# balazs-bamer/cdpr-simulation

Measured on AMD Instinct MI355X. Metric: CDPR sim-steps/sec (whole node), 65 536 parallel 8-cable robots, 1 ms dt, higher is better.
Workload: dtype f32

## Files before the change

cdpr-simulation_amd/csrc/cdpr_engine_launch.hip:

```cpp
#include "cdpr_engine_internal.hpp"

namespace cdpr_host {

double sim_time(uint64_t step, double dt) {
  const int64_t dt_ns = (int64_t)std::llround(dt * 1e9);
  const int64_t now_ns = (int64_t)step * dt_ns;
  return (double)(now_ns / 1000000000LL) + (double)(now_ns % 1000000000LL) * 1e-9;
}

uint64_t publish_mask(const cdpr_engine* h, int k, double& last) {
  uint64_t mask = 0;
  last = h->prev_publish;
  if (h->cfg.publish_period == 0.0) {
    if (k > 0 && h->step + (uint64_t)k > 1) last = sim_time(h->step + (uint64_t)k - 1, h->cfg.dt);
    mask = (k >= 64) ? ~0ull : ((1ull << k) - 1ull);
    return h->step == 0 ? (mask & ~1ull) : mask;
  }
  for (int j = 0; j < k; ++j) {
    const double now = sim_time(h->step + (uint64_t)j, h->cfg.dt);
    if ((now - last) > h->cfg.publish_period) {
      last = now;
      if (j < 64) mask |= (1ull << j);
    }
  }
  return mask;
}

void advance_clock(cdpr_engine* h, int k, int launches) {
  (void)publish_mask(h, k, h->prev_publish);
  if (!h->plan.general && h->mode != kModeForce) h->pid_calls = sat_pid_calls(h->pid_calls + k - (h->step == 0 ? 1 : 0));
  h->step += (uint64_t)k;
  h->launches += (uint64_t)launches;
}

static void set_weight_row(const cdpr_engine* h, StepArgs& a, int slot) {
  memcpy(a.wrow, &h->wtab_host[(h->plan.per_robot || h->mode == kModeVelocity) ? 0 : 1][slot * (kWin + 2)], sizeof a.wrow);
}

LaunchShape launch_shape(const cdpr_engine* h, int k, bool steady, const Schedule* sched) {
  LaunchShape s;
  s.steps = k;
  s.first_world = h->step == 0;
  s.scheduled = sched != nullptr;
  s.steady = steady;
  return s;
}
StepKernel step_kernel_of(const cdpr_engine* h, const PlannedKernel& pk) {
  const uint32_t n = h->n;
  switch (pk.id) {
    case KernelId::StepSingle: return pick_step_kernel(true, n, h->plan.fk, h->plan.td);
    case KernelId::StepMulti: return pick_step_kernel(false, n, h->plan.fk, h->plan.td);
    case KernelId::Lowreg: return pick_lowreg_kernel(n, h->plan.td);
    case KernelId::OnestepPersist: return pick_onestep_persist_kernel(n, h->plan.fk, h->plan.td);
    case KernelId::Split: return pick_split_kernel(n);
    case KernelId::Onestep: return pick_onestep_kernel(n, h->plan.fk, h->plan.td);
    case KernelId::PhysStep: return pick_phys_kernel(n, h->plan.fk, h->plan.td, kPhysStep);
    case KernelId::Rollout: return pick_rollout_kernel(n, h->plan.fk, h->plan.td);
    case KernelId::PhysRollout: return pick_phys_kernel(n, h->plan.fk, h->plan.td, kPhysRollout);
    case KernelId::PrSingle: return pick_pr_kernel(true, false, false, n, h->plan.fk, h->plan.td);
    case KernelId::PrLowreg: return pick_pr_kernel(true, false, true, n, h->plan.fk, h->plan.td);
    case KernelId::PrSplit: return pick_pr_split_kernel(n);
    case KernelId::PrMulti: return pick_pr_kernel(false, false, false, n, h->plan.fk, h->plan.td);
    case KernelId::PrRollout: return pick_pr_kernel(false, true, false, n, h->plan.fk, h->plan.td);
    case KernelId::PairSingle: return pick_pair_kernel(true, n, h->plan.fk, h->plan.td);
    case KernelId::PairMulti: return pick_pair_kernel(false, n, h->plan.fk, h->plan.td);
    case KernelId::PairStream: return pick_pair_stream_kernel(n, h->mode == kModeVelocity);
    case KernelId::Cable: return pick_cable_kernel(n, h->plan.fk, h->plan.td);
    default: return nullptr;
  }
}
StepKernel select_step_kernel(const cdpr_engine* h, int k, bool steady) { return step_kernel_of(h, planned_kernel(h->plan, launch_shape(h, k, steady))); }
static bool pair_stream_steady(const cdpr_engine* h, const StepArgs& a, const Schedule* sched) {
  return h->step != 0 && h->mode != kModeForce && a.pid_calls >= a.nbuf && h->cfg.publish_period == 0.0 && !a.dbg && !a.travel_on &&
         !(a.vel_limit > 0.f) && !a.unilateral && a.effort >= 0.f && a.clamp_cmd && !(sched && sched->ready);
}
static bool split_steady_launch(const cdpr_engine* h, const PlannedKernel& pk, const StepArgs& a) {
  return pk.id == KernelId::Split && h->split_steady && !h->plan.per_robot && h->step != 0 && h->mode != kModeForce && a.pid_calls != 0 &&
         a.pid_calls >= a.nbuf && h->cfg.publish_period == 0.0 && !a.dbg && !a.travel_on;
}
uint32_t step_block_threads(const cdpr_engine* h, int k) { return planned_kernel(h->plan, launch_shape(h, k)).block; }

static StepArgs handle_args(const cdpr_engine* h, const void* record) {
  StepArgs a = h->base;
  a.state = h->d_state;
  a.obs = h->d_obs;
  a.dbg = h->dbg ? h->d_dbg : nullptr;
  a.geom = h->d_geom;
  a.batch = h->batch;
  a.stride = h->stride;
  a.obs_step_stride = record ? (size_t)h->n_obs * h->stride : 0;
  return a;
}

static StepArgs fast_path_args(const cdpr_engine* h, const void* record, const Schedule* sched) {
  StepArgs a = handle_args(h, record);
  if (h->plan.per_robot) {
    copy_pid(h->pid_vel, a);
    copy_pid_alt(h->pid_pos, a.alt);
    a.cmd = h->d_target;
    a.meta = h->d_mode;
  } else {
    copy_pid(h->mode == kModeVelocity ? h->pid_vel : h->pid_pos, a);
    a.cmd = h->cmd[cmd_kind_of_mode(h->mode)].latched();
    a.flags = h->mode == kModeVelocity ? kFlagActualIsVelocity : h->mode == kModeForce ? kFlagForceMode : 0u;
  }
  if (sched) {
    a.flags |= kFlagPublishAll;
    a.sched_refresh = sched->refresh;
    a.sched_stride = (size_t)h->batch * h->n;
    a.sched_ready = sched->ready;
    a.fault = sched->fault;
  }
  return a;
}

int warm_first_launch(cdpr_engine* h) {
  if (h->plan.general || h->plan.fp64) return CDPR_OK;
  if (const char* w = std::getenv("CDPR_NO_WARM_LAUNCH"))
    if (w[0] == '1') return CDPR_OK;
  const uint32_t rows = 64;
  const std::vector<float4> s = home_state(h, rows);
  DevBuf st, ob, cm, mt;
  HIP_TRY(h, mt.alloc(rows));
  HIP_TRY(h, hipMemsetAsync(mt.p, (int)(kMetaPosition | (20u << kMetaCallShift)), rows, h->stream));
  HIP_TRY(h, st.alloc(s.size() * sizeof(float4)));
  HIP_TRY(h, ob.alloc((size_t)h->n_obs * rows * sizeof(float4)));
  HIP_TRY(h, cm.alloc((size_t)rows * h->n * sizeof(float)));
  HIP_TRY(h, hipMemcpyAsync(st.p, s.data(), s.size() * sizeof(float4), hipMemcpyHostToDevice, h->stream));
  HIP_TRY(h, hipMemsetAsync(cm.p, 0, (size_t)rows * h->n * sizeof(float), h->stream));
  StepArgs a = h->base;
  a.state = st.as<float4>();
  a.obs = ob.as<float4>();
  a.cmd = cm.as<float>();
  a.dbg = nullptr;
  a.geom = h->d_geom;
  a.batch = h->plan.lane_cable ? (h->n <= 4 ? 16u : 8u) : h->plan.lane_pair ? 32u : 64u;
  a.stride = rows;
  a.nsteps = 1;
  a.obs_step_stride = 0;
  a.flags = 0u;
  a.publish_mask = 1ull;
  copy_pid(h->plan.per_robot ? h->pid_vel : h->pid_pos, a);
  copy_pid_alt(h->pid_pos, a.alt);
  a.meta = mt.as<uint8_t>();
  a.pid_calls = kCallSat;
  a.ring_slot = 0;
  set_weight_row(h, a, 0);
  hipLaunchKernelGGL(select_step_kernel(h, 1), dim3(1), dim3(step_block_threads(h, 1)), 0, h->stream, a);
  HIP_TRY(h, hipGetLastError());
  if (planned_kernel(h->plan, launch_shape(h, 1)).id == KernelId::Split && h->split_steady) {
    for (const bool vel : {false, true}) {
      copy_pid(vel ? h->pid_vel : h->pid_pos, a);
      hipLaunchKernelGGL(pick_split_steady_kernel(h->n, vel), dim3(1), dim3(128), 0, h->stream, a);
      HIP_TRY(h, hipGetLastError());
    }
  }
  HIP_TRY(h, wait_stream(h));
  return CDPR_OK;
}

static int launch_step(cdpr_engine* h, StepKernel kern, uint32_t robots_per_block, dim3 block, const StepArgs& a, uint32_t max_grid = 0) {
  const uint32_t B = a.batch;
  const uint32_t chunk = (h->plan.chunk && B > h->plan.chunk) ? h->plan.chunk : B;
  const uint32_t pieces = (B + chunk - 1u) / chunk;
  const uint32_t each = (((B + pieces - 1u) / pieces) + 63u) & ~63u;
  int launches = 0;
  for (uint32_t first = 0; first < B; first += each, ++launches) {
    StepArgs c = a;
    c.batch = std::min(each, B - first);
    c.state = a.state + first;
    c.obs = a.obs + first;
    if (a.cmd) c.cmd = a.cmd + (size_t)first * h->n;
    if (a.dbg) c.dbg = a.dbg + (size_t)first * CDPR_PID_DEBUG_AXES;
    if (a.meta) c.meta = a.meta + first;
    uint32_t grid = (c.batch + robots_per_block - 1u) / robots_per_block;
    if (max_grid && grid > max_grid) grid = max_grid;
    hipLaunchKernelGGL(kern, dim3(grid), block, 0, h->stream, c);
  }
  return launches;
}

static void flush_hot(cdpr_engine* h) {
  if (!h->d_rec || !h->plan.gen_hot) return;
  GenFlushArgs fa{};
  fa.rec = h->d_rec, fa.rstride = h->stride, fa.batch = h->batch, fa.lay = h->glay, fa.nbuf = std::max(h->gpid[0].nbuf, 1);
  hipLaunchKernelGGL(cdpr_gen_flush_hot_kernel, dim3((h->batch + 255u) / 256u), dim3(256), 0, h->stream, fa);
}

static hipError_t reset_block(cdpr_engine* h, int which) {
  const GenLayout& L = h->glay;
  flush_hot(h);
  hipError_t e1 = hipMemsetAsync(h->d_rec + (size_t)L.block_a(which, 0) * h->stride * 4, 0, (size_t)L.pid_slots() * h->stride * 16, h->stream);
  if (e1 != hipSuccess || L.pid_rows() == 0) return e1;
  return hipMemsetAsync(h->d_rec + ((size_t)L.slots() * 4 + (size_t)L.block_b(which, 0)) * h->stride, 0, (size_t)L.pid_rows() * h->stride * 4, h->stream);
}

static hipError_t reset_block64(cdpr_engine* h, int which) {
  for (uint32_t i = 0; i < h->n; ++i) {
    hipError_t e1 = hipMemsetAsync(h->d_state64 + (size_t)f64_hold_row((int)h->n, (int)i, which, hold_win(h)) * h->stride, 0, (size_t)hold_pid_rows(hold_win(h)) * h->stride * sizeof(double),
                                   h->stream);
    if (e1 != hipSuccess) return e1;
  }
  return hipSuccess;
}

static int latch_per_robot(cdpr_engine* h, int kind, const float* pending, const uint8_t* mask) {
  const CmdKind& K = kCmdKind[kind];
  const dim3 grid((h->batch + 255u) / 256u), block(256);
  if (h->plan.fp64) {
    LatchF64Args lf{};
    lf.mask = mask;
    lf.meta = h->d_mode;
    lf.pending = pending;
    lf.target = h->d_target;
    lf.state = h->d_state64;
    lf.stride = h->stride;
    lf.batch = h->batch;
    lf.n = h->n;
    lf.new_mode = K.meta;
    lf.hold = h->plan.hold64 ? 1u : 0u;
    lf.win = (uint32_t)win64(h);
    lf.hold_win = (uint32_t)hold_win(h);
    hipLaunchKernelGGL(cdpr_latch_f64_kernel, grid, block, 0, h->stream, lf);
  } else if (!h->plan.general) {
    LatchFastArgs lf{};
    lf.mask = mask;
    lf.meta = h->d_mode;
    lf.pending = pending;
    lf.target = h->d_target;
    lf.hot = h->d_state + (size_t)(plat_slots(h->plan.fk) + 5 * cable_pairs((int)h->n)) * h->stride;
    lf.stride = h->stride;
    lf.batch = h->batch;
    lf.n = h->n;
    lf.hot_rows = (uint32_t)((cable_pairs((int)h->n) + 1) / 2);
    lf.new_mode = K.meta;
    hipLaunchKernelGGL(cdpr_latch_fast_kernel, grid, block, 0, h->stream, lf);
  } else {
    flush_hot(h);
    GenLatchArgs la{};
    la.mask = mask;
    la.mode = h->d_mode;
    la.pending = pending;
    la.latched = h->cmd[kind].d[0];
    la.rec = h->d_rec;
    la.rstride = h->stride;
    la.batch = h->batch;
    la.n = h->n;
    la.reset_pid = K.reset_pid;
    la.lay = h->glay;
    la.new_mode = K.mode;
    hipLaunchKernelGGL(cdpr_gen_latch_kernel, grid, block, 0, h->stream, la);
  }
  HIP_TRY(h, hipGetLastError());
  return CDPR_OK;
}

static int latch_pending(cdpr_engine* h, bool& reset_pid) {
  for (CmdChannel& c : h->cmd) {
    if (c.pending && c.ready_wait) {
      HIP_TRY(h, hipStreamWaitEvent(h->stream, c.ready_wait, 0));
      c.ready_wait = nullptr;
    }
  }
  bool touched[kCmdKinds] = {false, false, false};
  for (int k = 0; k < kCmdKinds; ++k) {
    CmdChannel& c = h->cmd[k];
    if (!c.pending) continue;
    const CmdKind& K = kCmdKind[k];
    if (h->plan.per_robot) {
      const bool in_place = c.sched_rows != nullptr;
      if (int rc = latch_per_robot(h, k, in_place ? c.sched_rows : c.d[1].p, in_place ? c.sched_mask : (c.masked ? c.d_mask.p : nullptr))) return rc;
      touched[k] = !in_place;
    } else {
      if (c.ext[1]) {
        c.ext[0] = c.ext[1];
        c.ext[1] = nullptr;
      } else {
        c.d[0].swap(c.d[1]);
        c.ext[0] = nullptr;
        touched[k] = true;
      }
      if (K.reset_pid >= 0) {
        reset_pid = (h->mode != K.mode);
        if (h->plan.general && reset_pid) HIP_TRY(h, reset_block(h, K.reset_pid));
        if (h->plan.hold64 && reset_pid) HIP_TRY(h, reset_block64(h, K.reset_pid));
      }
      h->mode = K.mode;
    }
    c.pending = c.masked = false;
    c.have = true;
  }
  for (CmdChannel& c : h->cmd) c.sched_rows = nullptr;
  for (int k = 0; k < kCmdKinds; ++k) {
    CmdChannel& c = h->cmd[k];
    if (!touched[k] || !h->copy_stream) continue;
    if (!c.free_ev) HIP_TRY(h, hipEventCreateWithFlags(&c.free_ev, hipEventDisableTiming));
    HIP_TRY(h, hipEventRecord(c.free_ev, h->stream));
    c.free_ev_set = true;
  }
  return CDPR_OK;
}

static int run_steps_general(cdpr_engine* h, int nsteps, int per_launch, void* record) {
  if (h->step + (uint64_t)nsteps >= (1ull << 31)) {
    h->err = "general controller path: world-step counter would pass 2^31";
    return CDPR_ERR_UNSUPPORTED;
  }
  StepArgs a = handle_args(h, record);
  a.cmd = nullptr;
  a.pid_calls = 0;
  copy_pid(h->pid_pos, a);
  GenCtl g = general_ctl(h);
  if (h->plan.gen_split || h->plan.gen_lean) per_launch = 1;
  return run_chain(h, nsteps, per_launch, record, h->d_obs, [&](ChainStep& s) {
    const PlannedKernel pk = planned_kernel(h->plan, launch_shape(h, s.k));
    const bool gsplit = pk.id == KernelId::GenSplit, glean = pk.id == KernelId::GenLean;
    GenKernel kern = gsplit ? pick_gen_split11(h->n) : glean ? pick_gen_lean11(h->n) : pick_gen_kernel(h->n, h->plan.fk, h->plan.td, false, h->glay.nb > 11, pk.id == KernelId::GenOne);
    h->last_kernel = pk;
    a.nsteps = s.k;
    a.flags = s.first_flag;
    g.now_step = (int)h->step;
    if (s.record) a.obs = static_cast<float4*>(s.record);
    a.publish_mask = s.publish_mask;
    hipLaunchKernelGGL(kern, dim3((h->batch + 63u) / 64u), dim3((gsplit || glean) ? 128 : 64), 0, h->stream, a, g);
    HIP_TRY(h, hipGetLastError());
    return (int)CDPR_OK;
  });
}

constexpr int kGraphChunk = 10;

int run_steps(cdpr_engine* h, int nsteps, int per_launch, void* record, const Schedule* sched) {
  if (!h) return CDPR_ERR_INVALID;
  if (nsteps < 0 || per_launch < 1 || (per_launch > 64 && !sched)) {
    h->err = "nsteps must be >= 0 and steps_per_launch in 1..64";
    return CDPR_ERR_INVALID;
  }
  if (nsteps == 0) return CDPR_OK;
  if (set_device(h) != CDPR_OK) return CDPR_ERR_DEVICE;

  bool reset_pid = false;
  if (int rc = latch_pending(h, reset_pid)) return rc;
  if (h->plan.general) return run_steps_general(h, nsteps, per_launch, record);
  if (h->plan.fp64) return run_steps_f64(h, nsteps, per_launch, reset_pid, record);

  if (reset_pid) {
    h->pid_calls = 0;
    const int P = plat_slots(h->plan.fk);
    HIP_TRY(h, hipMemsetAsync(h->d_state + (size_t)P * h->stride, 0, (size_t)ctrl_slots((int)h->n) * h->stride * sizeof(float4), h->stream));
  }
  StepArgs a = fast_path_args(h, record, sched);
  const uint32_t mode_flags = a.flags;
  const uint32_t robots_per_block = h->plan.lane_cable ? (h->n <= 4 ? 16u : 8u) : h->plan.lane_pair ? 32u : 64u;
  const dim3 grid((h->batch + robots_per_block - 1u) / robots_per_block);

  return run_chain(h, nsteps, per_launch, record, h->d_obs, [&](ChainStep& s) {
    const int k = s.k;
    a.nsteps = k;
    a.flags = mode_flags | s.first_flag;
    a.pid_calls = sat_pid_calls(h->pid_calls);
    a.ring_slot = ring_slot_of(h->step);
    const PlannedKernel pk = planned_kernel(h->plan, launch_shape(h, sched ? std::max(k, 2) : k, pair_stream_steady(h, a, sched), sched));
    StepKernel kern = step_kernel_of(h, pk);
    h->last_variant = split_steady_launch(h, pk, a) ? 1 : 0;
    if (h->last_variant) kern = pick_split_steady_kernel(h->n, h->mode == kModeVelocity);
    h->last_kernel = pk;
    const bool stream = pk.id == KernelId::PairStream;
    set_weight_row(h, a, stream ? 0 : a.ring_slot);
    if (s.record) a.obs = static_cast<float4*>(s.record);
    a.publish_mask = sched ? 0 : s.publish_mask;

    const bool steady = !record && !sched && h->use_graphs && (size_t)h->batch * h->n <= 131072u && !s.first_flag &&
                        (h->plan.per_robot || a.pid_calls == kCallSat || h->mode == kModeForce) && h->cfg.publish_period == 0.0 && s.left >= kGraphChunk * k;
    if (steady) {
      const GraphKey key{(void*)kern, a.cmd, k, a.ring_slot, a.flags};
      hipGraphExec_t exec = h->graphs.find(key);
      if (!exec)
        exec = h->graphs.capture(h->stream, key, [&] {
          bool launched = true;
          for (int j = 0; j < kGraphChunk; ++j) {
            StepArgs aj = a;
            aj.ring_slot = (a.ring_slot + j * k) % kWin;
            set_weight_row(h, aj, stream ? 0 : aj.ring_slot);
            hipLaunchKernelGGL(kern, grid, dim3(pk.block), 0, h->stream, aj);
            launched = launched && (hipGetLastError() == hipSuccess);
          }
          return launched;
        });
      if (exec) {
        HIP_TRY(h, hipGraphLaunch(exec, h->stream));
        s.used = kGraphChunk * k, s.launches = kGraphChunk;
        return (int)CDPR_OK;
      }
      h->use_graphs = false;
    }
    s.launches = launch_step(h, kern, robots_per_block, dim3(pk.block), a, (h->plan.persist && k == 1 && !h->plan.per_robot) ? h->persist_grid : 0u);
    HIP_TRY(h, hipGetLastError());
    return (int)CDPR_OK;
  });
}

int scheduled_update(cdpr_engine* h, uint32_t kind, int nsteps, int refresh_steps, const float* d_commands, const uint32_t* d_ready, const uint8_t* d_masks,
                     void* d_record, size_t record_bytes) {
  if (kind > 2u) {
    h->err = "cdpr_update_scheduled_kind: kind must be CDPR_COMMAND_VELOCITY, _POSITION or _FORCE";
    return CDPR_ERR_INVALID;
  }
  if (nsteps < 0 || refresh_steps < 1 || !d_commands) {
    h->err = "cdpr_update_scheduled: nsteps >= 0, refresh_steps >= 1 and the command schedule are required";
    return CDPR_ERR_INVALID;
  }
  if (d_masks && !h->plan.per_robot) {
    h->err = "cdpr_update_scheduled_kind: robot masks need a handle created with per_robot_commands = 1";
    return CDPR_ERR_UNSUPPORTED;
  }
  if (h->cfg.publish_period != 0.0 && d_record) {
    h->err = "cdpr_update_scheduled: a trajectory record needs publish_period == 0 (every step published)";
    return CDPR_ERR_UNSUPPORTED;
  }
  const size_t image = image_bytes(h);
  if (d_record && record_bytes < image * (size_t)nsteps) {
    h->err = "cdpr_update_scheduled: record buffer smaller than nsteps observable images";
    return CDPR_ERR_INVALID;
  }
  if (nsteps == 0) return CDPR_OK;
  if (set_device(h) != CDPR_OK) return CDPR_ERR_DEVICE;
  if (d_ready && !h->h_fault) {
    HIP_TRY(h, h->h_fault.alloc(sizeof(uint32_t), hipHostMallocMapped | hipHostMallocCoherent));
    *h->h_fault = 0u;
    HIP_TRY(h, hipHostGetDevicePointer((void**)&h->d_fault, h->h_fault, 0));
  }
  auto record_at = [&](int done) -> void* { return d_record ? static_cast<char*>(d_record) + (size_t)done * image : nullptr; };
  const size_t batch_floats = (size_t)h->batch * h->n;
  CmdChannel& c = h->cmd[kind];
  const int nbatches = (nsteps + refresh_steps - 1) / refresh_steps;
  auto stage_batch = [&](int j) {
    const float* rows = d_commands + (size_t)j * batch_floats;
    if (h->plan.per_robot) {
      c.sched_rows = rows;
      c.sched_mask = d_masks ? d_masks + (size_t)j * h->batch : nullptr;
    } else {
      c.ext[1] = rows;
    }
    c.pending = true;
    c.masked = false;
  };
  if (h->plan.per_robot && c.pending) {
    h->err = "cdpr_update_scheduled_kind: a command of the same kind is still pending on this per-robot handle; step it in with cdpr_update first";
    return CDPR_ERR_INVALID;
  }
  struct Unstage {
    cdpr_engine* h; CmdChannel& c; bool ok = false;
    ~Unstage() {
// ... 47 lines not shown
```

cdpr-simulation_amd/csrc/cdpr_onestep_kernel.hpp:

```cpp
#pragma once
#include "cdpr_step_kernel.hpp"

namespace cdpr {

CDPR_DEV void row_to_lds(const float4* src, float4* dst_row) {
  __builtin_amdgcn_global_load_lds((const __attribute__((address_space(1))) void*)src, (__attribute__((address_space(3))) void*)dst_row, 16, 0, 0);
}


template <int NP, bool PR = false, bool FULL = false>
CDPR_DEV void pid_pairs(const StepArgs& a, int calls, bool is_vel, const v2f (&desired)[NP], const v2f (&actual)[NP], const v2f (&win)[NP][kWin],
                        v2f (&ierr)[NP], v2f (&f)[NP], v2f (&e_new)[NP], float& dbg_p, float& dbg_i, float& dbg_d, bool is_force = false) {
  const PidCoef c = pid_coef<PR>(a, is_vel);
  const bool run = (!PR || calls != 0) && !is_force;
  const bool full = FULL || calls >= c.nbuf;
  const float (&wt)[kWin + 2] = a.wrow;
  v2f error[NP], acc[NP];
#pragma unroll
  for (int k = 0; k < NP; ++k) {
    error[k] = desired[k] - actual[k];
    acc[k] = splat(wt[kWin]) * error[k];
  }
#pragma unroll
  for (int j = 0; j < kWin; ++j) {
// ... 72 lines not shown
  const bool first_world = (a.flags & kFlagFirstWorldStep) != 0u;
  const bool run_pid = !first_world && !force_mode && a.pid_calls != 0;
  bool staged = false;

  for (;;) {
  size_t st = st0;
  uint32_t goff = 0;
  if (PERSIST) asm volatile("" : "+s"(st), "+v"(goff));
  const float* const geo = lds + goff;
  const StepArgs a = block_args<PERSIST>(a_in);
  v2f desired[NP];
#pragma unroll
  for (int k = 0; k < NP; ++k) desired[k] = splat(0.f);
  const float* cp = a.cmd + (size_t)rr * N;
  if (!kCmdLds || force_mode) {
#pragma unroll
    for (int i = 0; i < N; ++i) {
      if (i & 1)
        desired[i / 2].y = cp[i];
      else
        desired[i / 2].x = cp[i];
    }
  }
  __builtin_amdgcn_fence(__ATOMIC_RELEASE, "wavefront");
  __builtin_amdgcn_wave_barrier();
  __builtin_amdgcn_fence(__ATOMIC_ACQUIRE, "wavefront");

  Platform s;
  unpack_platform(p0, p1, p2, p3.x, s);
  float fkx = p3.y, fky = p3.z, fkz = p3.w, fkqx = p4.x, fkqy = p4.y, fkqz = p4.z, fkqw = p4.w;

  {
    float keep = (s.px + s.qy) + (s.vy + s.wz) + fkqw;
#pragma unroll
    for (int k = 0; k < NP; ++k) keep += desired[k].x + desired[k].y;
    asm volatile("" ::"v"(keep));
    if (run_pid && !staged) {
#pragma unroll
      for (int j = 0; j < kCtrl; ++j)
        row_to_lds(reinterpret_cast<const float4*>(reinterpret_cast<const char*>(a.state + (size_t)(P + j) * st) + off), &stage[j][0]);
      if (kCmdLds) {
#pragma unroll
        for (int g = 0; g < kCmdRows; ++g) row_to_lds(reinterpret_cast<const float4*>(cp) + g, &stage[kCtrl + g][0]);
      }
    }
  }

  const uint32_t nblk = blk + gridDim.x;
  const bool more = PERSIST && nblk < nblocks;
  uint32_t nr = 0, nrr = 0;
  f32x4 n0 = {0.f, 0.f, 0.f, 0.f}, n1 = n0, n2 = n0, n3 = n0, n4 = {0.f, 0.f, 0.f, 1.f};
  if (PERSIST && more) {
    nr = nblk * 64u + lane;
    nrr = (nr < a.batch) ? nr : (a.batch - 1u);
    const uint32_t noff = nrr * 16u;
    n0 = load_slot_untracked(a.state, st, 0, noff), n1 = load_slot_untracked(a.state, st, 1, noff);
    n2 = load_slot_untracked(a.state, st, 2, noff), n3 = load_slot_untracked(a.state, st, 3, noff);
    if (FK) n4 = load_slot_untracked(a.state, st, 4, noff);
  }

  CDPR_STAMP(1);
  v2f len[NP], q[NP], qd[NP], jac[NP][6];
  {
    v2f l0[NP];
    ik_pairs<N, true>(geo, s.px, s.py, s.pz, s.qx, s.qy, s.qz, s.qw, len, jac, l0);
#pragma unroll
    for (int k = 0; k < NP; ++k) {
      q[k] = l0[k] - len[k];
      qd[k] = -fma2(s.wz, jac[k][5], fma2(s.wy, jac[k][4], fma2(s.wx, jac[k][3],
                    fma2(s.vz, jac[k][2], fma2(s.vy, jac[k][1], splat(s.vx) * jac[k][0])))));
    }
  }
  const bool publish = (a.publish_mask & 1ull) != 0ull;
  if (publish && live) {
    store_slot(a.obs, st, 0, woff, make_float4(s.px, s.py, s.pz, s.qx));
    store_slot(a.obs, st, 1, woff, make_float4(s.qy, s.qz, s.qw, s.vx));
    store_slot(a.obs, st, 2, woff, make_float4(s.vy, s.vz, s.wx, s.wy));
#pragma unroll
    for (int g = 0; g < G; ++g) {
      const int k0 = 2 * g, k1 = (2 * g + 1 < NP) ? 2 * g + 1 : 2 * g;
      const bool has = (2 * g + 1 < NP);
      store_slot(a.obs, st, 4 + g, woff, make_float4(q[k0].x, q[k0].y, has ? q[k1].x : 0.f, has ? q[k1].y : 0.f));
      store_slot(a.obs, st, 4 + G + g, woff, make_float4(qd[k0].x, qd[k0].y, has ? qd[k1].x : 0.f, has ? qd[k1].y : 0.f));
    }
  }

  CDPR_STAMP(2);
  float fk_res = 0.f;
  int fk_it = 0;
  v2f jest[NP][6];
  if (FK) {
    v2f elen[NP], unused[NP];
    bool active = true;
    for (int it = 0; it < a.fk_iters; ++it) {
      ik_pairs<N, false>(geo, fkx, fky, fkz, fkqx, fkqy, fkqz, fkqw, elen, jest, unused);
      v2f res[NP];
      v2f rm = splat(0.f);
#pragma unroll
      for (int k = 0; k < NP; ++k) {
        res[k] = len[k] - elen[k];
        rm = max2(rm, abs2(res[k]));
      }
      active = active && !(fmaxf(rm.x, rm.y) < a.fk_tol);
      float g[6];
      jt_times<NP>(jest, res, g);
      normal_solve<NP>(jest, a.fk_lambda, g);
      if (active) {
        fkx += g[0];
        fky += g[1];
        fkz += g[2];
        quat_apply_rotvec(fkqx, fkqy, fkqz, fkqw, g[3], g[4], g[5]);
        ++fk_it;
      }
    }
    ik_pairs<N, false>(geo, fkx, fky, fkz, fkqx, fkqy, fkqz, fkqw, elen, jest, unused);
    v2f rm = splat(0.f);
#pragma unroll
    for (int k = 0; k < NP; ++k) rm = max2(rm, abs2(len[k] - elen[k]));
    fk_res = fmaxf(rm.x, rm.y);
  }

  CDPR_STAMP(3);
  v2f f[NP], e_new[NP], ierr[NP];
#pragma unroll
  for (int k = 0; k < NP; ++k) {
    f[k] = splat(0.f);
    e_new[k] = splat(0.f);
    ierr[k] = splat(0.f);
  }
  float dbg_p = 0.f, dbg_i = 0.f, dbg_d = 0.f;
  bool dbg_wrote = false;
  if (run_pid) {
    __builtin_amdgcn_s_waitcnt(0x0F70);
    __builtin_amdgcn_fence(__ATOMIC_ACQUIRE, "wavefront");
    CDPR_STAMP(4);
    if (kCmdLds) {
#pragma unroll
      for (int g = 0; g < kCmdRows; ++g) {
        const float4 v = stage[kCtrl + g][lane];
        desired[2 * g] = (v2f){v.x, v.y};
        desired[2 * g + 1] = (v2f){v.z, v.w};
      }
    }
    v2f win[NP][kWin];
#pragma unroll
    for (int k = 0; k < NP; ++k) {
#pragma unroll
      for (int m = 0; m < 5; ++m) {
        const float4 w = stage[5 * k + m][lane];
        win[k][2 * m] = (v2f){w.x, w.y};
        win[k][2 * m + 1] = (v2f){w.z, w.w};
      }
    }
#pragma unroll
    for (int g = 0; g < NH; ++g) {
      const float4 h = stage[5 * NP + g][lane];
      ierr[2 * g] = (v2f){h.x, h.y};
      if (2 * g + 1 < NP) ierr[2 * g + 1] = (v2f){h.z, h.w};
    }
    const bool actual_is_vel = (a.flags & kFlagActualIsVelocity) != 0u;
    v2f actual[NP];
#pragma unroll
    for (int k = 0; k < NP; ++k) actual[k] = actual_is_vel ? qd[k] : q[k];
    const int ring_slot = a.ring_slot;
    pid_pairs<NP>(a, a.pid_calls, actual_is_vel, desired, actual, win, ierr, f, e_new, dbg_p, dbg_i, dbg_d);
    dbg_wrote = true;
    if (live) {
#pragma unroll
      for (int m = 0; m < 5; ++m) {
        if (m == (ring_slot >> 1)) {
#pragma unroll
          for (int k = 0; k < NP; ++k) CDPR_STORE_STATE(a.state, st, P + 5 * k + m, woff, ring_row(win[k], m, e_new[k], ring_slot));
        }
      }
#pragma unroll
      for (int g = 0; g < NH; ++g) {
        const int k1 = (2 * g + 1 < NP) ? 2 * g + 1 : 2 * g;
        CDPR_STORE_STATE(a.state, st, P + 5 * NP + g, woff, make_float4(ierr[2 * g].x, ierr[2 * g].y, ierr[k1].x, ierr[k1].y));
      }
    }
  }

  if (force_mode && !first_world) {
#pragma unroll
    for (int k = 0; k < NP; ++k) f[k] = desired[k];
  }

  if (PERSIST && more) {
    const uint32_t noff = nrr * 16u;
    if (run_pid) {
#pragma unroll
      for (int j = 0; j < kCtrl; ++j)
        row_to_lds(reinterpret_cast<const float4*>(reinterpret_cast<const char*>(a.state + (size_t)(P + j) * st) + noff), &stage[j][0]);
      if (kCmdLds) {
        const float* ncp = a.cmd + (size_t)nrr * N;
#pragma unroll
        for (int g = 0; g < kCmdRows; ++g) row_to_lds(reinterpret_cast<const float4*>(ncp) + g, &stage[kCtrl + g][0]);
      }
    }
  }

  CDPR_STAMP(5);
  v2f applied[NP];
  int td_flag = 0;
  if (TD) {
    v2f df[NP];
#pragma unroll
    for (int k = 0; k < NP; ++k) df[k] = f[k] - splat(a.td_mid);
    float g[6];
    if (FK) {
      jt_times<NP>(jest, df, g);
      normal_solve<NP, false>(jest, 0.f, g);
    } else {
      jt_times<NP>(jac, df, g);
      normal_solve<NP, false>(jac, 0.f, g);
    }
#pragma unroll
    for (int k = 0; k < NP; ++k) {
      v2f t = splat(a.td_mid);
#pragma unroll
      for (int c = 0; c < 6; ++c) t = fma2(g[c], FK ? jest[k][c] : jac[k][c], t);
      const v2f tc = max2(min2(t, splat(a.td_max)), splat(a.td_min));
      td_flag |= (tc.x != t.x) ? 1 : 0;
      if (2 * k + 1 < N) td_flag |= (tc.y != t.y) ? 1 : 0;
      applied[k] = tc;
    }
  } else {
#pragma unroll
    for (int k = 0; k < NP; ++k) applied[k] = f[k];
  }
  setforce_limits<NP>(a, qd, applied);

  if (a.dbg && live) write_pid_topic(a.dbg + (size_t)r * 9, dbg_wrote, dbg_wrote, dbg_p, dbg_i, dbg_d, desired[0].x, applied[0].x);
  if (publish && live) {
    store_slot(a.obs, st, 3, woff, make_float4(s.wz, fk_res, (float)fk_it, pack_flags(td_flag, travel_mask<N>(a, q))));
#pragma unroll
    for (int g = 0; g < G; ++g) {
      const int k0 = 2 * g, k1 = (2 * g + 1 < NP) ? 2 * g + 1 : 2 * g;
      const bool has = (2 * g + 1 < NP);
      store_slot(a.obs, st, 4 + 2 * G + g, woff,
                make_float4(applied[k0].x, applied[k0].y, has ? applied[k1].x : 0.f, has ? applied[k1].y : 0.f));
    }
  }

  CDPR_STAMP(6);
  {
    v2f tens[NP];
#pragma unroll
    for (int k = 0; k < NP; ++k) {
      tens[k] = fma2(-a.damping, qd[k], applied[k]);
      if (a.unilateral) tens[k] = max2(tens[k], splat(0.f));
    }
    if (FK) {
      uint32_t again = 0;
      asm volatile("" : "+v"(again));
      v2f len2[NP], l02[NP];
      ik_pairs<N, false>(lds + again, s.px, s.py, s.pz, s.qx, s.qy, s.qz, s.qw, len2, jac, l02);
    }
    float w[6];
    jt_times<NP>(jac, tens, w);
    w[0] = a.fgx - w[0];
    w[1] = a.fgy - w[1];
    w[2] = a.fgz - w[2];
    w[3] = -w[3];
    w[4] = -w[4];
    w[5] = -w[5];
    integrate(a, s, w);
  }
  if (PERSIST && more) {
    constexpr int kDmaOps = kCtrl + kCmdRows;
    static_assert(kDmaOps < 64, "vmcnt is a 6-bit counter");
    if (run_pid)
      __builtin_amdgcn_s_waitcnt(vmcnt_imm(kDmaOps));
    else
      __builtin_amdgcn_s_waitcnt(vmcnt_imm(0));
    asm volatile("" : "+a"(n0), "+a"(n1), "+a"(n2), "+a"(n3), "+a"(n4));
  }
  if (live) {
    CDPR_STORE_STATE(a.state, st, 0, woff, make_float4(s.px, s.py, s.pz, s.qx));
    CDPR_STORE_STATE(a.state, st, 1, woff, make_float4(s.qy, s.qz, s.qw, s.vx));
    CDPR_STORE_STATE(a.state, st, 2, woff, make_float4(s.vy, s.vz, s.wx, s.wy));
    CDPR_STORE_STATE(a.state, st, 3, woff, make_float4(s.wz, fkx, fky, fkz));
    if (FK) CDPR_STORE_STATE(a.state, st, 4, woff, make_float4(fkqx, fkqy, fkqz, fkqw));
  }
  CDPR_STAMP(7);
  if (!(PERSIST && more)) break;
  blk = nblk;
  r = nr;
  rr = nrr;
  live = r < a.batch;
  off = rr * 16u, woff = r * 16u;
  p0 = make_float4(n0.x, n0.y, n0.z, n0.w), p1 = make_float4(n1.x, n1.y, n1.z, n1.w), p2 = make_float4(n2.x, n2.y, n2.z, n2.w);
  p3 = make_float4(n3.x, n3.y, n3.z, n3.w), p4 = make_float4(n4.x, n4.y, n4.z, n4.w);
  staged = run_pid;
  }
}

#ifndef CDPR_CTL_LOAD_DELAY
#define CDPR_CTL_LOAD_DELAY 8
#endif
#ifndef CDPR_SPLIT_PRIO
#define CDPR_SPLIT_PRIO 1
#endif
#ifdef CDPR_STAMPS
#define CDPR_SPLIT_STAMP(i)                                                                                          \
  do {                                                                                                               \
    __builtin_amdgcn_sched_barrier(0);                                                                               \
    if (a.stamps && lane == 0) a.stamps[(size_t)blockIdx.x * 8 + (i)] = __builtin_amdgcn_s_memrealtime();           \
    __builtin_amdgcn_sched_barrier(0);                                                                               \
  } while (0)
#else
#define CDPR_SPLIT_STAMP(i) do { } while (0)
#endif
#if defined(CDPR_STAMPS) && defined(CDPR_STAMPS_ITER)
#define CDPR_CTL_STAMP(i) do { } while (0)
#else
#define CDPR_CTL_STAMP(i) CDPR_SPLIT_STAMP(i)
#endif

template <int N, int XS, int ES, bool RAISED = true>
CDPR_DEV void split_estimator_wave(const StepArgs& a, float* geo, float gval, uint32_t lane, bool live, size_t st, uint32_t off, uint32_t woff,
                                   const float4& p0, const float4& p1, const float4& p3, const v2f* x_force, v2f* x_tension, float* x_est) {
  constexpr int NP = cable_pairs(N);
#if defined(CDPR_STAMPS) && defined(CDPR_STAMPS_CLOCK)
  const unsigned long long clk0 = __builtin_amdgcn_s_memtime();
#endif
#if CDPR_SPLIT_PRIO == 1 || CDPR_SPLIT_PRIO == 4
  if (RAISED) __builtin_amdgcn_s_setprio(3);
#elif CDPR_SPLIT_PRIO == 3 || CDPR_SPLIT_PRIO == 5
  if (RAISED) __builtin_amdgcn_s_setprio(2);
#endif
  const float4 p4 = load_slot(a.state, st, 4, off);
  if (lane < NP * kGeomFloatsPerPair) geo[lane] = gval;
  __builtin_amdgcn_fence(__ATOMIC_RELEASE, "wavefront");
  __builtin_amdgcn_wave_barrier();
  __builtin_amdgcn_fence(__ATOMIC_ACQUIRE, "wavefront");
  float fkx = p3.y, fky = p3.z, fkz = p3.w, fkqx = p4.x, fkqy = p4.y, fkqz = p4.z, fkqw = p4.w;
  v2f len[NP];
  {
    v2f jac[NP][6], l0[NP];
    ik_pairs<N, false>(geo, p0.x, p0.y, p0.z, p0.w, p1.x, p1.y, p1.z, len, jac, l0);
  }
  float fk_res = 0.f;
  int fk_it = 0;
  v2f jest[NP][6];
  {
    v2f elen[NP], unused[NP];
    bool active = true;
    for (int it = 0; it < a.fk_iters; ++it) {
      ik_pairs<N, false>(geo, fkx, fky, fkz, fkqx, fkqy, fkqz, fkqw, elen, jest, unused);
      v2f res[NP];
      v2f rm = splat(0.f);
#pragma unroll
      for (int k = 0; k < NP; ++k) {
        res[k] = len[k] - elen[k];
        rm = max2(rm, abs2(res[k]));
      }
      active = active && !(fmaxf(rm.x, rm.y) < a.fk_tol);
      float g[6];
      jt_times<NP>(jest, res, g);
      normal_solve<NP>(jest, a.fk_lambda, g);
      if (active) {
        fkx += g[0];
        fky += g[1];
        fkz += g[2];
        quat_apply_rotvec(fkqx, fkqy, fkqz, fkqw, g[3], g[4], g[5]);
        ++fk_it;
      }
#ifdef CDPR_STAMPS_ITER
      if (it < 3) {
        asm volatile("" ::"v"(fkqw));
        __builtin_amdgcn_sched_barrier(0);
        if (a.stamps && lane == 0) a.stamps[(size_t)blockIdx.x * 8 + 4 + it] = __builtin_amdgcn_s_memrealtime();
        __builtin_amdgcn_sched_barrier(0);
      }
#endif
    }
    ik_pairs<N, false>(geo, fkx, fky, fkz, fkqx, fkqy, fkqz, fkqw, elen, jest, unused);
    v2f rm = splat(0.f);
#pragma unroll
    for (int k = 0; k < NP; ++k) rm = max2(rm, abs2(len[k] - elen[k]));
    fk_res = fmaxf(rm.x, rm.y);
  }
  if (live) store_slot_aux<CDPR_SPLIT_PLAT_AUX>(a.state, st, 4, woff, make_float4(fkqx, fkqy, fkqz, fkqw));
  CDPR_SPLIT_STAMP(1);
  v2f td_l[6][3];
  float td_invd[6];
  normal_matrix_pk<NP, false>(jest, 0.f, td_l);
  chol_factor_pk(td_l, td_invd);
  __builtin_amdgcn_s_waitcnt(0xC07F);
  __builtin_amdgcn_s_barrier();
  CDPR_SPLIT_STAMP(2);
  __builtin_amdgcn_fence(__ATOMIC_ACQUIRE, "workgroup");
  v2f f[NP], df[NP], t_out[NP];
#pragma unroll
  for (int k = 0; k < NP; ++k) {
    f[k] = x_force[k * XS + lane];
    df[k] = f[k] - splat(a.td_mid);
  }
  int td_flag = 0;
  {
    float g[6];
    jt_times<NP>(jest, df, g);
    chol_apply_pk(td_l, td_invd, g);
#pragma unroll
    for (int k = 0; k < NP; ++k) {
      v2f t = splat(a.td_mid);
#pragma unroll
      for (int c = 0; c < 6; ++c) t = fma2(g[c], jest[k][c], t);
      const v2f tc = max2(min2(t, splat(a.td_max)), splat(a.td_min));
      td_flag |= (tc.x != t.x) ? 1 : 0;
      if (2 * k + 1 < N) td_flag |= (tc.y != t.y) ? 1 : 0;
      t_out[k] = tc;
    }
  }
#pragma unroll
  for (int k = 0; k < NP; ++k) x_tension[k * XS + lane] = t_out[k];
  x_est[0 * ES + lane] = fkx;
  x_est[1 * ES + lane] = fky;
  x_est[2 * ES + lane] = fkz;
  x_est[3 * ES + lane] = fk_res;
  x_est[4 * ES + lane] = (float)fk_it;
  x_est[5 * ES + lane] = (float)td_flag;
  __builtin_amdgcn_fence(__ATOMIC_RELEASE, "workgroup");
  __builtin_amdgcn_s_waitcnt(0xC07F);
  CDPR_SPLIT_STAMP(3);
#if defined(CDPR_STAMPS) && defined(CDPR_STAMPS_CLOCK)
  if (a.stamps && lane == 0) a.stamps[(size_t)blockIdx.x * 8 + 7] = __builtin_amdgcn_s_memtime() - clk0;
#endif
  __builtin_amdgcn_s_barrier();
}

template <int N, bool PR, bool STEADY, bool VEL>
CDPR_DEV void split_controller_wave(const StepArgs& a, float* geo, float gval, uint32_t lane, uint32_t r, uint32_t rr, bool live, size_t st, uint32_t off,
                                    uint32_t woff, const float4& p0, const float4& p1, const float4& p2, const float4& p3, v2f* x_force, const v2f* x_tension,
                                    const float* x_est) {
  static_assert(!(STEADY && PR), "the steady instantiation serves uniform handles");
  constexpr int NP = cable_pairs(N);
  constexpr int P = plat_slots(true);
  constexpr int G = joint_groups(N);
  constexpr int NH = (NP + 1) / 2;
#if CDPR_SPLIT_PRIO == 2 || CDPR_SPLIT_PRIO == 5
  __builtin_amdgcn_s_setprio(3);
#endif
#if CDPR_CTL_LOAD_DELAY > 0
  __builtin_amdgcn_s_sleep(CDPR_CTL_LOAD_DELAY);
#endif
  float4 wraw[NP][5], hraw[NH];
#pragma unroll
  for (int k = 0; k < NP; ++k) {
#pragma unroll
    for (int m = 0; m < 5; ++m) wraw[k][m] = load_slot(a.state, st, P + 5 * k + m, off);
  }
#pragma unroll
  for (int g = 0; g < NH; ++g) hraw[g] = load_slot(a.state, st, P + 5 * NP + g, off);
  v2f desired[NP];
#pragma unroll
  for (int k = 0; k < NP; ++k) desired[k] = splat(0.f);
  const float* cp = a.cmd + (size_t)rr * N;
  if (N % 4 == 0) {
#pragma unroll
    for (int g = 0; g < N / 4; ++g) {
      const float4 v = reinterpret_cast<const float4*>(cp)[g];
      desired[2 * g] = (v2f){v.x, v.y};
      desired[2 * g + 1] = (v2f){v.z, v.w};
    }
  } else {
#pragma unroll
    for (int i = 0; i < N; ++i) {
      if (i & 1)
        desired[i / 2].y = cp[i];
      else
        desired[i / 2].x = cp[i];
    }
  }
  if (lane < NP * kGeomFloatsPerPair) geo[lane] = gval;
  __builtin_amdgcn_fence(__ATOMIC_RELEASE, "wavefront");
  __builtin_amdgcn_wave_barrier();
  __builtin_amdgcn_fence(__ATOMIC_ACQUIRE, "wavefront");

  Platform s;
  unpack_platform(p0, p1, p2, p3.x, s);

  v2f len[NP], q[NP], qd[NP], jac[NP][6];
  {
    v2f l0[NP];
    ik_pairs<N, true>(geo, s.px, s.py, s.pz, s.qx, s.qy, s.qz, s.qw, len, jac, l0);
#pragma unroll
    for (int k = 0; k < NP; ++k) {
      q[k] = l0[k] - len[k];
      qd[k] = -fma2(s.wz, jac[k][5], fma2(s.wy, jac[k][4], fma2(s.wx, jac[k][3],
                    fma2(s.vz, jac[k][2], fma2(s.vy, jac[k][1], splat(s.vx) * jac[k][0])))));
    }
  }
  const bool publish = STEADY || (a.publish_mask & 1ull) != 0ull;
  if (publish && live) {
    store_slot(a.obs, st, 0, woff, make_float4(s.px, s.py, s.pz, s.qx));
    store_slot(a.obs, st, 1, woff, make_float4(s.qy, s.qz, s.qw, s.vx));
    store_slot(a.obs, st, 2, woff, make_float4(s.vy, s.vz, s.wx, s.wy));
#pragma unroll
    for (int g = 0; g < G; ++g) {
      const int k0 = 2 * g, k1 = (2 * g + 1 < NP) ? 2 * g + 1 : 2 * g;
      const bool has = (2 * g + 1 < NP);
      store_slot(a.obs, st, 4 + g, woff, make_float4(q[k0].x, q[k0].y, has ? q[k1].x : 0.f, has ? q[k1].y : 0.f));
      store_slot(a.obs, st, 4 + G + g, woff, make_float4(qd[k0].x, qd[k0].y, has ? qd[k1].x : 0.f, has ? qd[k1].y : 0.f));
    }
  }

  v2f f[NP], e_new[NP], ierr[NP];
#pragma unroll
  for (int k = 0; k < NP; ++k) {
    f[k] = splat(0.f);
    e_new[k] = splat(0.f);
    ierr[k] = (k & 1) ? (v2f){hraw[k / 2].z, hraw[k / 2].w} : (v2f){hraw[k / 2].x, hraw[k / 2].y};
  }
  float dbg_p = 0.f, dbg_i = 0.f, dbg_d = 0.f;
  bool dbg_wrote = false;
  const bool first_world = !STEADY && (a.flags & kFlagFirstWorldStep) != 0u;
  uint32_t meta = 0u;
  if (PR) meta = a.meta[rr];
  const int calls = PR ? (int)(meta >> kMetaCallShift) : a.pid_calls;
  if (PR && live && !first_world) a.meta[r] = (uint8_t)((meta & kMetaModeMask) | ((uint32_t)min(calls + 1, (int)kMetaCallMax) << kMetaCallShift));
  const bool force_mode = !STEADY && !PR && (a.flags & kFlagForceMode) != 0u;
  if (force_mode && !first_world) {
#pragma unroll
    for (int k = 0; k < NP; ++k) f[k] = desired[k];
  } else if (STEADY || (!first_world && (PR || calls != 0))) {
    v2f win[NP][kWin];
#pragma unroll
    for (int k = 0; k < NP; ++k) {
#pragma unroll
      for (int m = 0; m < 5; ++m) {
        win[k][2 * m] = (v2f){wraw[k][m].x, wraw[k][m].y};
        win[k][2 * m + 1] = (v2f){wraw[k][m].z, wraw[k][m].w};
      }
    }
    const bool actual_is_vel = STEADY ? VEL : PR ? ((meta & kMetaModeMask) == kMetaVelocity) : ((a.flags & kFlagActualIsVelocity) != 0u);
    v2f actual[NP];
#pragma unroll
    for (int k = 0; k < NP; ++k) actual[k] = actual_is_vel ? qd[k] : q[k];
    const int ring_slot = a.ring_slot;
    const bool is_force = PR && (meta & kMetaModeMask) == kMetaForce;
#if CDPR_SPLIT_PRIO == 3 || CDPR_SPLIT_PRIO == 4
    __builtin_amdgcn_s_setprio(3);
#endif
    pid_pairs<NP, PR, STEADY>(a, calls, actual_is_vel, desired, actual, win, ierr, f, e_new, dbg_p, dbg_i, dbg_d, is_force);
    dbg_wrote = (!PR || calls != 0) && !is_force;
    if (live) {
#pragma unroll
      for (int m = 0; m < 5; ++m) {
        if (m == (ring_slot >> 1)) {
          if (!STEADY) {
#pragma unroll
            for (int k = 0; k < NP; ++k) CDPR_STORE_STATE(a.state, st, P + 5 * k + m, woff, ring_row(win[k], m, e_new[k], ring_slot));
          } else if (ring_slot & 1) {
#pragma unroll
            for (int k = 0; k < NP; ++k) CDPR_STORE_STATE(a.state, st, P + 5 * k + m, woff, make_float4(win[k][2 * m].x, win[k][2 * m].y, e_new[k].x, e_new[k].y));
          } else {
#pragma unroll
            for (int k = 0; k < NP; ++k) CDPR_STORE_STATE(a.state, st, P + 5 * k + m, woff, make_float4(e_new[k].x, e_new[k].y, win[k][2 * m + 1].x, win[k][2 * m + 1].y));
          }
        }
      }
#pragma unroll
      for (int g = 0; g < NH; ++g) {
        const int k1 = (2 * g + 1 < NP) ? 2 * g + 1 : 2 * g;
        CDPR_STORE_STATE(a.state, st, P + 5 * NP + g, woff, make_float4(ierr[2 * g].x, ierr[2 * g].y, ierr[k1].x, ierr[k1].y));
      }
    }
  }
#pragma unroll
  for (int k = 0; k < NP; ++k) x_force[k * 64 + lane] = f[k];
  __builtin_amdgcn_fence(__ATOMIC_RELEASE, "workgroup");
  __builtin_amdgcn_s_waitcnt(0xC07F);
  CDPR_CTL_STAMP(4);
#if CDPR_SPLIT_PRIO >= 3
  __builtin_amdgcn_s_setprio(0);
#endif
  __builtin_amdgcn_s_barrier();
  __builtin_amdgcn_s_barrier();
  CDPR_CTL_STAMP(5);
  __builtin_amdgcn_fence(__ATOMIC_ACQUIRE, "workgroup");
  v2f applied[NP];
#pragma unroll
  for (int k = 0; k < NP; ++k) applied[k] = x_tension[k * 64 + lane];
  const float fkx = x_est[0 * 64 + lane], fky = x_est[1 * 64 + lane], fkz = x_est[2 * 64 + lane], fk_res = x_est[3 * 64 + lane],
              fk_it = x_est[4 * 64 + lane], td_flag = x_est[5 * 64 + lane];
  setforce_limits<NP>(a, qd, applied);
  if (!STEADY && a.dbg && live) write_pid_topic(a.dbg + (size_t)r * 9, dbg_wrote, dbg_wrote, dbg_p, dbg_i, dbg_d, desired[0].x, applied[0].x);
  if (publish && live) {
    store_slot(a.obs, st, 3, woff, make_float4(s.wz, fk_res, fk_it, (!STEADY && a.travel_on) ? pack_flags((int)td_flag, travel_mask<N>(a, q)) : td_flag));
#pragma unroll
    for (int g = 0; g < G; ++g) {
      const int k0 = 2 * g, k1 = (2 * g + 1 < NP) ? 2 * g + 1 : 2 * g;
      const bool has = (2 * g + 1 < NP);
      store_slot(a.obs, st, 4 + 2 * G + g, woff,
                 make_float4(applied[k0].x, applied[k0].y, has ? applied[k1].x : 0.f, has ? applied[k1].y : 0.f));
    }
  }
  {
    v2f tens[NP];
#pragma unroll
    for (int k = 0; k < NP; ++k) {
      tens[k] = fma2(-a.damping, qd[k], applied[k]);
      if (a.unilateral) tens[k] = max2(tens[k], splat(0.f));
    }
    float w[6];
    jt_times<NP>(jac, tens, w);
    w[0] = a.fgx - w[0];
    w[1] = a.fgy - w[1];
    w[2] = a.fgz - w[2];
    w[3] = -w[3];
    w[4] = -w[4];
    w[5] = -w[5];
    integrate(a, s, w);
  }
  if (live) {
    store_slot_aux<CDPR_SPLIT_PLAT_AUX>(a.state, st, 0, woff, make_float4(s.px, s.py, s.pz, s.qx));
    store_slot_aux<CDPR_SPLIT_PLAT_AUX>(a.state, st, 1, woff, make_float4(s.qy, s.qz, s.qw, s.vx));
    store_slot_aux<CDPR_SPLIT_PLAT_AUX>(a.state, st, 2, woff, make_float4(s.vy, s.vz, s.wx, s.wy));
    store_slot_aux<CDPR_SPLIT_PLAT_AUX>(a.state, st, 3, woff, make_float4(s.wz, fkx, fky, fkz));
  }
  CDPR_CTL_STAMP(6);
}

template <int N, bool PR, bool STEADY, bool VEL>
CDPR_DEV void split_kernel_body(const StepArgs& a) {
  constexpr int NP = cable_pairs(N);
  __shared__ __attribute__((aligned(16))) float lds[2][NP * kGeomFloatsPerPair];
  __shared__ v2f x_force[NP][64];
  __shared__ v2f x_tension[NP][64];
  __shared__ float x_est[6][64];

  const uint32_t swap = __builtin_popcount(blockIdx.x & a.split_swap) & 1u;
  const uint32_t wave = (threadIdx.x >> 6) ^ swap, lane = threadIdx.x & 63u;
  const uint32_t r = blockIdx.x * 64u + lane;
  const uint32_t rr = (r < a.batch) ? r : (a.batch - 1u);
  const bool live = r < a.batch;
  const size_t st = a.stride;
  const uint32_t off = rr * 16u, woff = r * 16u;
  float* const geo = lds[wave];

  if (wave == 0) CDPR_SPLIT_STAMP(0);
#ifdef CDPR_STAMPS
  if (a.stamps && lane == 0)
    reinterpret_cast<uint32_t*>(&a.stamps[(size_t)blockIdx.x * 8 + 7])[threadIdx.x >> 6] =
        (__builtin_amdgcn_s_getreg((16 - 1) << 11 | 4) & 0xffffu) | ((__builtin_amdgcn_s_getreg((4 - 1) << 11 | 20) & 0xfu) << 16);
#endif
  const float gval = (lane < NP * kGeomFloatsPerPair) ? a.geom[lane] : 0.f;
  const float4 p0 = load_slot(a.state, st, 0, off), p1 = load_slot(a.state, st, 1, off), p2 = load_slot(a.state, st, 2, off),
               p3 = load_slot(a.state, st, 3, off);
  if (wave == 0) {
    split_estimator_wave<N, 64, 64>(a, geo, gval, lane, live, st, off, woff, p0, p1, p3, &x_force[0][0], &x_tension[0][0], &x_est[0][0]);
    return;
  }
  split_controller_wave<N, PR, STEADY, VEL>(a, geo, gval, lane, r, rr, live, st, off, woff, p0, p1, p2, p3, &x_force[0][0], &x_tension[0][0], &x_est[0][0]);
}
template <int N, bool PR = false>
__global__ __launch_bounds__(128, 2) void cdpr_split_kernel(const StepArgs a) { split_kernel_body<N, PR, false, false>(a); }
template <int N, bool VEL>
__global__ __launch_bounds__(128, 2) void cdpr_split_steady_kernel(const StepArgs a) { split_kernel_body<N, false, true, VEL>(a); }

}
```

Before: 6.625 billion.

## Share estimator IK with controller wave and unroll fixed four-iteration FK Newton in steady kernel

In the steady split kernel, the estimator wave writes its inverse-kinematics cable lengths and Jacobian for the current state to LDS, and the controller wave reads them after a barrier instead of recomputing IK. The forward-kinematics Newton loop is also fully unrolled to exactly four iterations with no tolerance check. The steady path is now gated on fk_tolerance being 0 and fk_max_iterations being 4, so results stay identical. The trade is extra LDS, a cross-wave barrier that couples the two waves' timing, and fewer cases that take the steady kernel.

```diff
diff --git a/cdpr-simulation_amd/csrc/cdpr_engine_launch.hip b/cdpr-simulation_amd/csrc/cdpr_engine_launch.hip
--- a/cdpr-simulation_amd/csrc/cdpr_engine_launch.hip
+++ b/cdpr-simulation_amd/csrc/cdpr_engine_launch.hip
@@ -74,9 +74,12 @@
   return h->step != 0 && h->mode != kModeForce && a.pid_calls >= a.nbuf && h->cfg.publish_period == 0.0 && !a.dbg && !a.travel_on &&
          !(a.vel_limit > 0.f) && !a.unilateral && a.effort >= 0.f && a.clamp_cmd && !(sched && sched->ready);
 }
+static bool split_steady_handle(const cdpr_engine* h) {
+  return h->split_steady && !h->plan.per_robot && h->cfg.publish_period == 0.0 && h->cfg.fk_tolerance == 0.0 && h->cfg.fk_max_iterations == 4;
+}
 static bool split_steady_launch(const cdpr_engine* h, const PlannedKernel& pk, const StepArgs& a) {
-  return pk.id == KernelId::Split && h->split_steady && !h->plan.per_robot && h->step != 0 && h->mode != kModeForce && a.pid_calls != 0 &&
-         a.pid_calls >= a.nbuf && h->cfg.publish_period == 0.0 && !a.dbg && !a.travel_on;
+  return pk.id == KernelId::Split && split_steady_handle(h) && h->step != 0 && h->mode != kModeForce && a.pid_calls != 0 &&
+         a.pid_calls >= a.nbuf && !a.dbg && !a.travel_on;
 }
 uint32_t step_block_threads(const cdpr_engine* h, int k) { return planned_kernel(h->plan, launch_shape(h, k)).block; }
 
@@ -148,7 +151,7 @@
   set_weight_row(h, a, 0);
   hipLaunchKernelGGL(select_step_kernel(h, 1), dim3(1), dim3(step_block_threads(h, 1)), 0, h->stream, a);
   HIP_TRY(h, hipGetLastError());
-  if (planned_kernel(h->plan, launch_shape(h, 1)).id == KernelId::Split && h->split_steady) {
+  if (planned_kernel(h->plan, launch_shape(h, 1)).id == KernelId::Split && split_steady_handle(h)) {
     for (const bool vel : {false, true}) {
       copy_pid(vel ? h->pid_vel : h->pid_pos, a);
       hipLaunchKernelGGL(pick_split_steady_kernel(h->n, vel), dim3(1), dim3(128), 0, h->stream, a);
diff --git a/cdpr-simulation_amd/csrc/cdpr_onestep_kernel.hpp b/cdpr-simulation_amd/csrc/cdpr_onestep_kernel.hpp
--- a/cdpr-simulation_amd/csrc/cdpr_onestep_kernel.hpp
+++ b/cdpr-simulation_amd/csrc/cdpr_onestep_kernel.hpp
@@ -398,6 +398,13 @@
 #ifndef CDPR_SPLIT_PRIO
 #define CDPR_SPLIT_PRIO 1
 #endif
+#ifndef CDPR_STEADY_SHARED_IK
+#define CDPR_STEADY_SHARED_IK 1
+#endif
+#ifndef CDPR_STEADY_NEWTON_WRITTEN_OUT
+#define CDPR_STEADY_NEWTON_WRITTEN_OUT 1
+#endif
+constexpr int kIkRows = 7;
 #ifdef CDPR_STAMPS
 #define CDPR_SPLIT_STAMP(i)                                                                                          \
   do {                                                                                                               \
@@ -414,9 +421,10 @@
 #define CDPR_CTL_STAMP(i) CDPR_SPLIT_STAMP(i)
 #endif
 
-template <int N, int XS, int ES, bool RAISED = true>
+template <int N, int XS, int ES, bool RAISED = true, bool STEADY = false>
 CDPR_DEV void split_estimator_wave(const StepArgs& a, float* geo, float gval, uint32_t lane, bool live, size_t st, uint32_t off, uint32_t woff,
-                                   const float4& p0, const float4& p1, const float4& p3, const v2f* x_force, v2f* x_tension, float* x_est) {
+                                   const float4& p0, const float4& p1, const float4& p3, const v2f* x_force, v2f* x_tension, float* x_est,
+                                   v2f* x_ik = nullptr) {
   constexpr int NP = cable_pairs(N);
 #if defined(CDPR_STAMPS) && defined(CDPR_STAMPS_CLOCK)
   const unsigned long long clk0 = __builtin_amdgcn_s_memtime();
@@ -436,41 +444,78 @@
   {
     v2f jac[NP][6], l0[NP];
     ik_pairs<N, false>(geo, p0.x, p0.y, p0.z, p0.w, p1.x, p1.y, p1.z, len, jac, l0);
+    if (STEADY && CDPR_STEADY_SHARED_IK) {
+#pragma unroll
+      for (int k = 0; k < NP; ++k) {
+        x_ik[(kIkRows * k) * 64 + lane] = len[k];
+#pragma unroll
+        for (int c = 0; c < 6; ++c) x_ik[(kIkRows * k + 1 + c) * 64 + lane] = jac[k][c];
+      }
+      __builtin_amdgcn_fence(__ATOMIC_RELEASE, "workgroup");
+      __builtin_amdgcn_s_waitcnt(0xC07F);
+      __builtin_amdgcn_s_barrier();
+    }
   }
   float fk_res = 0.f;
   int fk_it = 0;
   v2f jest[NP][6];
   {
     v2f elen[NP], unused[NP];
-    bool active = true;
-    for (int it = 0; it < a.fk_iters; ++it) {
-      ik_pairs<N, false>(geo, fkx, fky, fkz, fkqx, fkqy, fkqz, fkqw, elen, jest, unused);
-      v2f res[NP];
-      v2f rm = splat(0.f);
-#pragma unroll
-      for (int k = 0; k < NP; ++k) {
-        res[k] = len[k] - elen[k];
-        rm = max2(rm, abs2(res[k]));
-      }
-      active = active && !(fmaxf(rm.x, rm.y) < a.fk_tol);
-      float g[6];
-      jt_times<NP>(jest, res, g);
-      normal_solve<NP>(jest, a.fk_lambda, g);
-      if (active) {
+    if (STEADY && CDPR_STEADY_NEWTON_WRITTEN_OUT) {
+#pragma unroll
+      for (int it = 0; it < 4; ++it) {
+        ik_pairs<N, false>(geo, fkx, fky, fkz, fkqx, fkqy, fkqz, fkqw, elen, jest, unused);
+        v2f res[NP];
+#pragma unroll
+        for (int k = 0; k < NP; ++k) res[k] = len[k] - elen[k];
+        float g[6];
+        jt_times<NP>(jest, res, g);
+        normal_solve<NP>(jest, a.fk_lambda, g);
         fkx += g[0];
         fky += g[1];
         fkz += g[2];
         quat_apply_rotvec(fkqx, fkqy, fkqz, fkqw, g[3], g[4], g[5]);
-        ++fk_it;
-      }
 #ifdef CDPR_STAMPS_ITER
-      if (it < 3) {
-        asm volatile("" ::"v"(fkqw));
-        __builtin_amdgcn_sched_barrier(0);
-        if (a.stamps && lane == 0) a.stamps[(size_t)blockIdx.x * 8 + 4 + it] = __builtin_amdgcn_s_memrealtime();
-        __builtin_amdgcn_sched_barrier(0);
-      }
-#endif
+        if (it < 3) {
+          asm volatile("" ::"v"(fkqw));
+          __builtin_amdgcn_sched_barrier(0);
+          if (a.stamps && lane == 0) a.stamps[(size_t)blockIdx.x * 8 + 4 + it] = __builtin_amdgcn_s_memrealtime();
+          __builtin_amdgcn_sched_barrier(0);
+        }
+#endif
+      }
+      fk_it = 4;
+    } else {
+      bool active = true;
+      for (int it = 0; it < a.fk_iters; ++it) {
+        ik_pairs<N, false>(geo, fkx, fky, fkz, fkqx, fkqy, fkqz, fkqw, elen, jest, unused);
+        v2f res[NP];
+        v2f rm = splat(0.f);
+#pragma unroll
+        for (int k = 0; k < NP; ++k) {
+          res[k] = len[k] - elen[k];
+          rm = max2(rm, abs2(res[k]));
+        }
+        active = active && !(fmaxf(rm.x, rm.y) < a.fk_tol);
+        float g[6];
+        jt_times<NP>(jest, res, g);
+        normal_solve<NP>(jest, a.fk_lambda, g);
+        if (active) {
+          fkx += g[0];
+          fky += g[1];
+          fkz += g[2];
+          quat_apply_rotvec(fkqx, fkqy, fkqz, fkqw, g[3], g[4], g[5]);
+          ++fk_it;
+        }
+#ifdef CDPR_STAMPS_ITER
+        if (it < 3) {
+          asm volatile("" ::"v"(fkqw));
+          __builtin_amdgcn_sched_barrier(0);
+          if (a.stamps && lane == 0) a.stamps[(size_t)blockIdx.x * 8 + 4 + it] = __builtin_amdgcn_s_memrealtime();
+          __builtin_amdgcn_sched_barrier(0);
+        }
+#endif
+      }
     }
     ik_pairs<N, false>(geo, fkx, fky, fkz, fkqx, fkqy, fkqz, fkqw, elen, jest, unused);
     v2f rm = splat(0.f);
@@ -530,7 +575,7 @@
 template <int N, bool PR, bool STEADY, bool VEL>
 CDPR_DEV void split_controller_wave(const StepArgs& a, float* geo, float gval, uint32_t lane, uint32_t r, uint32_t rr, bool live, size_t st, uint32_t off,
                                     uint32_t woff, const float4& p0, const float4& p1, const float4& p2, const float4& p3, v2f* x_force, const v2f* x_tension,
-                                    const float* x_est) {
+                                    const float* x_est, const v2f* x_ik = nullptr) {
   static_assert(!(STEADY && PR), "the steady instantiation serves uniform handles");
   constexpr int NP = cable_pairs(N);
   constexpr int P = plat_slots(true);
@@ -581,7 +626,19 @@
   v2f len[NP], q[NP], qd[NP], jac[NP][6];
   {
     v2f l0[NP];
-    ik_pairs<N, true>(geo, s.px, s.py, s.pz, s.qx, s.qy, s.qz, s.qw, len, jac, l0);
+    if (STEADY && CDPR_STEADY_SHARED_IK) {
+      __builtin_amdgcn_s_barrier();
+      __builtin_amdgcn_fence(__ATOMIC_ACQUIRE, "workgroup");
+#pragma unroll
+      for (int k = 0; k < NP; ++k) {
+        len[k] = x_ik[(kIkRows * k) * 64 + lane];
+#pragma unroll
+        for (int c = 0; c < 6; ++c) jac[k][c] = x_ik[(kIkRows * k + 1 + c) * 64 + lane];
+        l0[k] = *reinterpret_cast<const v2f*>(geo + k * kGeomFloatsPerPair + 12);
+      }
+    } else {
+      ik_pairs<N, true>(geo, s.px, s.py, s.pz, s.qx, s.qy, s.qz, s.qw, len, jac, l0);
+    }
 #pragma unroll
     for (int k = 0; k < NP; ++k) {
       q[k] = l0[k] - len[k];
@@ -727,6 +784,11 @@
   __shared__ v2f x_force[NP][64];
   __shared__ v2f x_tension[NP][64];
   __shared__ float x_est[6][64];
+  v2f* x_ik = nullptr;
+  if constexpr (STEADY && CDPR_STEADY_SHARED_IK) {
+    __shared__ v2f ik_rows_at_state[kIkRows * NP][64];
+    x_ik = &ik_rows_at_state[0][0];
+  }
 
   const uint32_t swap = __builtin_popcount(blockIdx.x & a.split_swap) & 1u;
   const uint32_t wave = (threadIdx.x >> 6) ^ swap, lane = threadIdx.x & 63u;
@@ -747,10 +809,10 @@
   const float4 p0 = load_slot(a.state, st, 0, off), p1 = load_slot(a.state, st, 1, off), p2 = load_slot(a.state, st, 2, off),
                p3 = load_slot(a.state, st, 3, off);
   if (wave == 0) {
-    split_estimator_wave<N, 64, 64>(a, geo, gval, lane, live, st, off, woff, p0, p1, p3, &x_force[0][0], &x_tension[0][0], &x_est[0][0]);
+    split_estimator_wave<N, 64, 64, true, STEADY>(a, geo, gval, lane, live, st, off, woff, p0, p1, p3, &x_force[0][0], &x_tension[0][0], &x_est[0][0], x_ik);
     return;
   }
-  split_controller_wave<N, PR, STEADY, VEL>(a, geo, gval, lane, r, rr, live, st, off, woff, p0, p1, p2, p3, &x_force[0][0], &x_tension[0][0], &x_est[0][0]);
+  split_controller_wave<N, PR, STEADY, VEL>(a, geo, gval, lane, r, rr, live, st, off, woff, p0, p1, p2, p3, &x_force[0][0], &x_tension[0][0], &x_est[0][0], x_ik);
 }
 template <int N, bool PR = false>
 __global__ __launch_bounds__(128, 2) void cdpr_split_kernel(const StepArgs a) { split_kernel_body<N, PR, false, false>(a); }
```

Measured after the change: 6.808 billion, median of 6. 2.8% higher.
